# NOAA-GFDL/GFDL_atmos_cubed_sphere

Hardware: AMD Instinct MI355X
Metric: c_sw+d_sw cell-updates/s (higher is better)
Workload: dtype f64; 1 GPU; doubly periodic 384x384x127 tile per GPU (C384L127-sized), nonhydrostatic, c_sw+d_sw pair, hord 10/10/10/10, nord=1, d4_bg=0.16; layout=1x1, halo=periodic copy, gridstruct=orthogonal + uniform (metric terms as scalars), build_id=3496e67435bd, launch=eager launches

## Files before the change

### gfdl_atmos_cubed_sphere_amd/csrc/csw_march.h

```cpp
#pragma once

#include "csw_kernel.h"
#include "tp2d_march.h"

namespace fv3 {

constexpr int kCswCols = 58;
constexpr int kCswLast = 60;

inline MarchDims make_csw_dims(const Grid &g, int tj) {
  MarchDims d;
  d.tj = tj;
  d.klist = nullptr;
  d.nk = 0;
  d.k_fast = 0;
  d.nstrips = (g.nx + 4 + kCswCols - 1) / kCswCols;
  d.nsegs = (g.ny + 4 + tj - 1) / tj;
  d.alt_nk = d.alt_ng = d.alt_tj = 0;
  d.set_box(0, d.nstrips, 0, d.nsegs);
  return d;
}

struct CswMetrics {
  vd cs, rs, cosau, rsinu, dy, sg3, sg1, dx, sg4, sg2, dxc, dyc, rac, fc;
  vd ra, sinau, rdxc, cosav, sinav, rdyc;
};
struct CswFields {
  vd u, v, dp, pt, w;
};

struct CswLevel {
  vd u0, u1, u2, u3;
  vd v0, v1, v2, v3;
// ... 12 lines not shown
  }
};

template <int KPW, int GM = 0, bool CS = false>
struct CswMarch {
#ifdef FV3_CSW_TWO_WAVES
  static constexpr int kTwoWavesPerSimd = 1;
#endif
  Grid g;
  CswArgs a;
  MarchDims md;
  int nkg;

  FV3_D void operator()(int gid) const {
    constexpr double a1 = 0.5625, a2 = -0.0625;
    int strip, seg, kg, tjw;
    md.decode_tj(gid, strip, seg, kg, tjw);
    const int is = g.is, ie = g.ie, js = g.js, je = g.je;
    const int ilo = is - 1 + strip * kCswCols - 3;
    auto cl = [](int v, int lo, int hi) { return v < lo ? lo : (v > hi ? hi : v); };
    const vl cA = make_lanes(cl(g.isd - ilo, 0, kW - 1), cl(g.ied - ilo, 0, kW - 1));
    const vl cV = make_lanes(cl(g.isd - ilo, 0, kW - 1), cl(g.ied + 1 - ilo, 0, kW - 1));
    int l2 = cl(ie + 2 - ilo, 0, kCswLast), l1 = cl(ie + 1 - ilo, 0, kCswLast);
    const int mw = CS ? a.mask_w : 0;
    const int l0 = mw ? (3 > mw + 1 - ilo ? 3 : mw + 1 - ilo) : 3;
    if (mw) {
      const int lm = g.npx - mw - 1 - ilo;
      l2 = l2 < lm ? l2 : lm;
      l1 = l1 < lm ? l1 : lm;
    }
    const int oJ0 = mw ? mw + 1 : g.jsd - 1, oJ1 = mw ? g.npy - mw - 1 : g.jed + 2;
    const int jA = js - 1 + seg * tjw;
    const int jB = (jA + tjw - 1 < je + 2) ? jA + tjw - 1 : je + 2;
    const bool nh = !a.hydrostatic;
    const double dt2 = a.dt2, dt4 = 0.5 * dt2;
    const long nAp = (long)g.nA();
    auto LA = [&](const double *p, int j, long shift = 0) { return vload(p, (long)g.iA(ilo, cl(j, g.jsd, g.jed)) + shift, cA); };
    auto LU = [&](const double *p, int j) { return vload(p, (long)g.iU(ilo, cl(j, g.jsd, g.jed + 1)), cA); };
    auto LV = [&](const double *p, int j) { return vload(p, (long)g.iV(ilo, cl(j, g.jsd, g.jed)), cV); };
    auto LB = [&](const double *p, int j) { return vload(p, (long)g.iB(ilo, cl(j, g.jsd, g.jed + 1)), cV); };
    const vb m_uc = lane_mask(is - ilo, ie + 1 - ilo);
    const vb m_vc = lane_mask(is - ilo, ie - ilo);
    const vm s1 = make_mask(l0, l1), s2 = make_mask(l0, l2);

    int kl[KPW];
    bool live[KPW];
    for (int m = 0; m < KPW; m++) {
      const int k = kg * KPW + m;
// ... 174 lines not shown
```

### gfdl_atmos_cubed_sphere_amd/csrc/dsw_fused.h

```cpp
#pragma once

#include "dsw_march.h"

#ifndef FV3_BF
#define FV3_BF 1
#endif
#ifndef FV3_MOM_3W
#define FV3_MOM_3W 1
#endif

namespace fv3 {

struct Tp2dShared {
  vd cx, xf, ar, rax;
  vd cy, yf;
  vd arj, cxj, ray;
  vd rrax, rray;
};

template <int HORD>
struct Tp2dField {
  static constexpr int ORD_IN = (HORD == 10) ? 8 : HORD;
  static constexpr int ORD_OU = HORD;
  PpmY<ORD_IN> ya;
// ... 43 lines not shown
    vd cy, yf;
    vd xfj, ra;
    vd ucj;
    vd rdxa, dyr, sg3, sg1;
    vd rdya0, rdya1, dxr, sg4, sg2;
  };

  FV3_D void operator()(int gid) const {
    if constexpr (FLUXES || !FV3_BF)
      run_general(gid);
    else
      run_bf(gid);
  }

  FV3_D void run_bf(int gid) const {
    int strip, seg, kk, tjw;
    md.decode_tj(gid, strip, seg, kk, tjw);
    const int k = md.klist ? md.klist[kk] : kk;
    const StripGeom s = make_strip(g, strip);
    const int ilo = s.ilo;
    const int jA = g.js + seg * tjw;
    const int jB = (jA + tjw - 1 < g.je) ? jA + tjw - 1 : g.je;
    const int rlast = jB + 3;
    const int lFx1 = (ilo + s.lC1 == g.ie) ? s.lC1 + 1 : s.lC1;
    const size_t oA = (size_t)k * g.nA(), oCX = (size_t)k * g.nCX(), oCY = (size_t)k * g.nCY();
    const size_t oFX = (size_t)k * g.nFX(), oFY = (size_t)k * g.nFY(), oCC = (size_t)k * g.nCC();
    const double *delp = a.delp + oA, *pt = a.pt + oA, *w = NH ? a.w + oA : nullptr;
    double *crx = a.crx + oCX, *xfx = a.xfx + oCX, *cry = a.cry + oCY, *yfx = a.yfx + oCY;
    double *mfx = a.mfx + oFX, *mfy = a.mfy + oFY;
    const int seg_last = (jB == g.je);
    const int rowA = (seg == 0) ? g.jsd : jA, rowB = seg_last ? g.jed : jB;
    const int lY0 = (strip == 0) ? s.lA0 : s.lC0, lY1 = (ilo + s.lC1 == g.ie) ? s.lA1 : s.lC1;
    const double dt = a.dt;
    const int mw = a.mask_w;
    const int oC0 = mw ? (s.lC0 > mw + 1 - ilo ? s.lC0 : mw + 1 - ilo) : s.lC0;
    const int oC1 = mw ? (s.lC1 < g.npx - mw - 1 - ilo ? s.lC1 : g.npx - mw - 1 - ilo) : s.lC1;
    const int oF1 = mw ? (lFx1 < g.npx - mw - 1 - ilo ? lFx1 : g.npx - mw - 1 - ilo) : lFx1;
    const int oJ0 = mw ? mw + 1 : g.jsd, oJ1 = mw ? g.npy - mw - 1 : g.jed + 1;
    const vm mCX = make_mask(s.lC0, lFx1), mCY = make_mask(lY0, lY1), mO = make_mask(oC0, oC1), mOF = make_mask(oC0, oF1),
             mC = make_mask(s.lC0, s.lC1);
    const bool wdamp = UNI && NH && a.lv.damp_w[k] > 1.E-5;
    const double damp4 = wdamp ? a.lv.damp_w[k] * g.da_min_c : 0., dd8 = a.kgb * fabs(a.dt);

    auto load_in = [&](int r) {
      In in;
      const long iA = (long)g.iA(ilo, r), iCX = (long)g.iCX(ilo, r);
// ... 359 lines not shown

  struct In {
    vd u1, v0, v1, dx1, dy0, dy1, ra, f0;
    vd ar, cx, xf, cy, yf;
    vd vc, uc, ukc, rdy, rdx, dv, dgu, dgv, rac;
  };

  FV3_D void operator()(int gid) const {
    if constexpr (FV3_BF)
      run_bf(gid);
    else
      run_general(gid);
  }

  FV3_D void run_bf(int gid) const {
    int strip, seg, kk, tjw;
    md.decode_tj(gid, strip, seg, kk, tjw);
    const int k = md.klist ? md.klist[kk] : kk;
    const StripGeom s = make_strip(g, strip);
    const int ilo = s.ilo;
    const int jA = g.js + seg * tjw;
    const int jB = (jA + tjw - 1 < g.je) ? jA + tjw - 1 : g.je;
    const int rlast = jB + 3;
    const int lFx1 = (ilo + s.lC1 == g.ie) ? s.lC1 + 1 : s.lC1;
    const double *u = a.u + (size_t)k * g.nU(), *v = a.v + (size_t)k * g.nV();
    const double *uc = a.uc + (size_t)k * g.nV(), *vc = a.vc + (size_t)k * g.nU();
    const double *dv = a.divg_d + (size_t)k * g.nB();
    const double *crx = a.crx + (size_t)k * g.nCX(), *xfx = a.xfx + (size_t)k * g.nCX();
    const double *cry = a.cry + (size_t)k * g.nCY(), *yfx = a.yfx + (size_t)k * g.nCY();
    double *uo = a.u_out + (size_t)k * g.nU(), *vo = a.v_out + (size_t)k * g.nV();
    double *dpc = a.delpc ? a.delpc + (size_t)k * g.nA() : nullptr;
    const double dt5 = 0.5 * a.dt, dt = a.dt;
    const int mw = CS ? a.mask_w : 0;
    const int oC0 = (CS && mw) ? (s.lC0 > mw + 1 - ilo ? s.lC0 : mw + 1 - ilo) : s.lC0;
    const int oC1 = (CS && mw) ? (s.lC1 < g.npx - mw - 1 - ilo ? s.lC1 : g.npx - mw - 1 - ilo) : s.lC1;
    const int oF1 = (CS && mw) ? (lFx1 < g.npx - mw - 1 - ilo ? lFx1 : g.npx - mw - 1 - ilo) : lFx1;
    const int oJ0 = (CS && mw) ? mw + 1 : g.jsd, oJ1 = (CS && mw) ? g.npy - mw - 1 : g.jed + 1;
// ... 431 lines not shown
```

### gfdl_atmos_cubed_sphere_amd/csrc/fv3_api.hip

```cpp
#include "../../include/fv3_mi355x.h"

#include <algorithm>
#include <cstdarg>
#include <deque>
#include <unordered_map>
#include <new>
#include <type_traits>

#include "csw_kernel.h"
#include "csw_march.h"
#include "cubed_csw.h"
#include "cubed_tp.h"
#include "cubed_tpf.h"
#include "cube_topo.h"
#include "cubed_dsw.h"
#include "cubed_damp.h"
#include "cubed_a2b.h"
#include "dsw_kernels.h"
#include "dsw_march.h"
#include "dsw_fused.h"
#include "fv3_common.h"
#include "fv3_launch.h"
#include "nh_kernels.h"
#include "nh_fast.h"
#include "nh_alt.h"
#include "neg_adj.h"
#include "subgrid_z.h"
#include "phys_update.h"
#include "held_suarez.h"
#include "reed_phys.h"
#include "kessler_phys.h"
#include "diag_kernels.h"
#include "remap_kernels.h"
#include "remap_fast.h"
#include "tracer_kernels.h"
// ... 13 lines not shown
struct CubePlanDev;
constexpr int kMarchTj = 48;
struct fv3_ctx {
  fv3_domain dom = {};
  Grid g = {};
  stream_t stream = {};
  stream_t stream2 = {};
  void *ev_fork = nullptr, *ev_join = nullptr;
  int lane = 0;
  void *ev_mid = nullptr;
  bool side_ok = false;
  struct LevSel { int *klist, *klist_m; int n_plain, n_damp, n_plain_m, n_rest_m; bool side_ok; } lev_sel[2] = {};
  int use_side = 1;
  int sponge_march = 1;
  int round_simds = 0;
  double *dev_metrics = nullptr;
  bool grid_ready = false;
  int *lev_i = nullptr;
  double *lev_d = nullptr;
  bool lev_ready = false;
  double *dp0 = nullptr;
  double *edge_dev = nullptr;
  EdgeCoef ec = {};
  bool dp0_ready = false;
  double *scratch[8] = {};
  double *ray_d = nullptr;
  struct RegEntry { const void *host; void *dev; size_t bytes; bool dev_current, host_current; };
  std::vector<RegEntry> *reg = nullptr;
  int reg_lazy = 0;
  long long reg_stat[4] = {};
// ... 498 lines not shown
  g.is = dom->is; g.ie = dom->ie; g.js = dom->js; g.je = dom->je;
  g.isd = dom->is - NG; g.ied = dom->ie + NG; g.jsd = dom->js - NG; g.jed = dom->je + NG;
  g.npx = dom->npx; g.npy = dom->npy; g.npz = dom->npz;
  g.nid = g.ied - g.isd + 1; g.njd = g.jed - g.jsd + 1; g.nx = g.ie - g.is + 1; g.ny = g.je - g.js + 1;
  g.grid_type = dom->grid_type;
  g.do_diss_est = dom->do_diss_est; g.prevent_diss_cooling = dom->prevent_diss_cooling;
  g.stretched_grid = dom->stretched_grid;
  g.lim_fac = dom->lim_fac;
  ctx_switches(c);
  *out = c;
  return 0;
}

extern "C" int fv3_comm_destroy(fv3_ctx *c);
static void cube_plans_free(fv3_ctx *c);
extern "C" int fv3_destroy(fv3_ctx *c) {
  if (!c) return 0;
  if (c->grp) {
    fv3_group *g = c->grp;
    (void)grp_pump(g, true);
    for (int m = 0; m < g->n; m++)
      if (g->m[m] == c) g->m[m] = nullptr;
    for (int m = 0; m < g->n; m++)
      if (g->m[m]) g->m[m]->grp = nullptr;
    g->n = 0;
    c->grp = nullptr;
  }
  const int guards = c->poison ? work_check_guards(c, "fv3_destroy") : 0;
  cube_plans_free(c);
  fv3_comm_destroy(c);
  if (c->dev_metrics) rt_free(c->dev_metrics);
  if (c->lev_i) rt_free(c->lev_i);
  if (c->lev_d) rt_free(c->lev_d);
  if (c->dp0) rt_free(c->dp0);
  if (c->akbk) rt_free(c->akbk);
  work_free(c, &c->remap_scr);
  if (c->ray_d) rt_free(c->ray_d);
  if (c->rff_d) rt_free(c->rff_d);
  delete c->reg;
  work_free(c, &c->trc_d);
  if (c->trc_i) rt_free(c->trc_i);
  if (c->ones_i) rt_free(c->ones_i);
  if (c->kord_tr_dev) rt_free(c->kord_tr_dev);
  if (c->edge_dev) rt_free(c->edge_dev);
  if (c->lev_ext_d) rt_free(c->lev_ext_d);
// ... 178 lines not shown
  RT(grp_stream_op(c, 2, dst, src, bytes, 0));
  return 0;
}
extern "C" int fv3_memset(fv3_ctx *c, void *dst, int value, size_t bytes) {
  RT(grp_stream_op(c, 1, dst, nullptr, bytes, value));
  return 0;
}
extern "C" int fv3_sync(fv3_ctx *c) {
  RT(rtf_sync(c ? c->stream : nullptr));
  if (c && c->poison) return work_check_guards(c, "fv3_sync");
  return 0;
}

extern "C" int fv3_grid_upload(fv3_ctx *c, const fv3_grid_host *h) {
  if (!c || !h) return fail("fv3_grid_upload: null argument");
  c->host_area.clear();
  c->global_area = 0.;
  Grid &g = c->g;
  const size_t nA = g.nA(), nU = g.nU(), nV = g.nV(), nB = g.nB();
  struct Item { const double *src; const double **dst; size_t n; };
  Item items[] = {
      {h->area, &g.area, nA}, {h->rarea, &g.rarea, nA}, {h->dxa, &g.dxa, nA}, {h->dya, &g.dya, nA},
      {h->rdxa, &g.rdxa, nA}, {h->rdya, &g.rdya, nA}, {h->cosa_s, &g.cosa_s, nA}, {h->rsin2, &g.rsin2, nA},
      {h->f0, &g.f0, nA},
      {h->dx, &g.dx, nU}, {h->rdx, &g.rdx, nU}, {h->dyc, &g.dyc, nU}, {h->rdyc, &g.rdyc, nU},
      {h->cosa_v, &g.cosa_v, nU}, {h->sina_v, &g.sina_v, nU}, {h->rsin_v, &g.rsin_v, nU},
      {h->divg_u, &g.divg_u, nU}, {h->del6_u, &g.del6_u, nU},
      {h->dy, &g.dy, nV}, {h->rdy, &g.rdy, nV}, {h->dxc, &g.dxc, nV}, {h->rdxc, &g.rdxc, nV},
      {h->cosa_u, &g.cosa_u, nV}, {h->sina_u, &g.sina_u, nV}, {h->rsin_u, &g.rsin_u, nV},
      {h->divg_v, &g.divg_v, nV}, {h->del6_v, &g.del6_v, nV},
// ... 44 lines not shown
  return 0;
}

extern "C" int fv3_grid_geom(const fv3_ctx *c) { return (c && c->grid_ready) ? c->g.geom : -1; }

static void lev_activate(fv3_ctx *c, int x) {
  const fv3_ctx::LevSel &ls = c->lev_sel[x];
  c->klist = ls.klist; c->n_plain = ls.n_plain; c->n_damp = ls.n_damp;
  c->klist_m = ls.klist_m; c->n_plain_m = ls.n_plain_m; c->n_rest_m = ls.n_rest_m;
  c->side_ok = ls.side_ok;
}

extern "C" int fv3_dsw_levels_upload(fv3_ctx *c, const fv3_dsw_levels *lv) {
  if (!c || !lv) return fail("fv3_dsw_levels_upload: null argument");
  const int npz = c->g.npz;
  if (!c->lev_i) RT(rt_malloc((void **)&c->lev_i, sizeof(int) * 4 * npz));
  if (!c->lev_d) RT(rt_malloc((void **)&c->lev_d, sizeof(double) * 5 * npz));
  const int *iv[4] = {lv->nord_k, lv->nord_v, lv->nord_w, lv->nord_t};
  const double *dv[5] = {lv->d2_divg, lv->damp_vt, lv->damp_w, lv->damp_t, lv->d_con_k};
  for (int n = 0; n < 4; n++) {
    for (int k = 0; k < npz; k++) {
      if (iv[n][k] < 0 || iv[n][k] > (n == 0 ? 3 : 2)) return fail("fv3_dsw_levels_upload: nord out of range at k=%d", k);
    }
    RT(rtf_h2d(c->lev_i + n * npz, iv[n], sizeof(int) * npz, c->stream));
  }
  for (int n = 0; n < 5; n++) RT(rtf_h2d(c->lev_d + n * npz, dv[n], sizeof(double) * npz, c->stream));
  {
    std::vector<int> ni(npz + 1);
    std::vector<double> nd(npz + 1);
    for (int k = 0; k < npz; k++) { ni[k] = lv->nord_v[k]; nd[k] = lv->damp_vt[k]; }
// ... 451 lines not shown
    case 11: RT(launch_w(c, "ppm_line", 1, PpmLineMarch<11>{h, cr, flux, n, which - 1})); break;
    case 12: RT(launch_w(c, "ppm_line", 1, PpmLineMarch<12>{h, cr, flux, n, which - 1})); break;
    case 1: RT(launch_w(c, "ppm_line", 1, PpmLineMarchLin<1>{h, cr, flux, n, which - 1, c->g.lim_fac})); break;
    case -1: RT(launch_w(c, "ppm_line", 1, PpmLineMarchLin<-1>{h, cr, flux, n, which - 1, c->g.lim_fac})); break;
    case 2: RT(launch_w(c, "ppm_line", 1, PpmLineMarchLin<2>{h, cr, flux, n, which - 1, c->g.lim_fac})); break;
    case -2: RT(launch_w(c, "ppm_line", 1, PpmLineMarchLin<-2>{h, cr, flux, n, which - 1, c->g.lim_fac})); break;
    case 3: RT(launch_w(c, "ppm_line", 1, PpmLineMarchLin<3>{h, cr, flux, n, which - 1, c->g.lim_fac})); break;
    case -3: RT(launch_w(c, "ppm_line", 1, PpmLineMarchLin<-3>{h, cr, flux, n, which - 1, c->g.lim_fac})); break;
    case 4: RT(launch_w(c, "ppm_line", 1, PpmLineMarchLin<4>{h, cr, flux, n, which - 1, c->g.lim_fac})); break;
    case -4: RT(launch_w(c, "ppm_line", 1, PpmLineMarchLin<-4>{h, cr, flux, n, which - 1, c->g.lim_fac})); break;
    default: return fail("fv3_ppm_line: hord=%d not supported -- " FV3_HORD_TABLE, iord);
  }
  return 0;
}

static void seg_report(const char *who, const MarchDims &d, int nlev) {
  static const int on = env_int("FV3_MI355X_DEBUG_SEGMENTS", 0);
  if (on)
    std::fprintf(stderr, "[fv3 segments] %s: %d level slots x %d strips x %d segments of %d rows; %d of the slots (spread evenly): %d segments of %d rows\n", who, nlev,
                 d.nstrips, d.nsegs, d.tj, d.alt_nk, d.alt_ng, d.alt_tj);
}
static int seg_rows(const fv3_ctx *c, int tj_conf, int nlev_slots) {
  const Grid &g = c->g;
  if (c->tj_fixed) return tj_conf;
  const int nstrips = num_strips(g);
  const long have = (long)nstrips * (nlev_slots > 0 ? nlev_slots : 1);
  const int want_segs = (int)((2048 + have - 1) / have);
  int tj = (g.ny + want_segs - 1) / want_segs;
  if (tj < 8) tj = 8;
  return tj < tj_conf ? tj : tj_conf;
}

template <class F>
static int dispatch_geom(int geom, F &&f) {
  switch (geom) {
    case 2: return f(std::integral_constant<int, 2>{});
    case 1: return f(std::integral_constant<int, 1>{});
    default: return f(std::integral_constant<int, 0>{});
  }
}

extern "C" int fv3_c_sw(fv3_ctx *c, double *delpc, const double *delp, double *ptc, const double *pt,
                        const double *u, const double *v, const double *w, double *uc, double *vc, double *ua,
                        double *va, double *wc, double *ut, double *vt, double *divg_d, int nord, double dt2,
                        int hydrostatic, int dord4) {
// ... 11 lines not shown
  kf.g = c->g;
  kf.a = CswArgs{delpc, ptc, wc, uc, vc, ua, va, ut, vt, divg_d, delp, pt, u, v, w, nord, hydrostatic, dt2};
  Dim3 grid;
  CswTile<TI, TJ>::grid_dims(c->g, grid.x, grid.y);
  grid.z = (unsigned)c->g.npz;
  RT(launch_p(c, "c_sw", grid, CswTile<TI, TJ>::lds_doubles, kf));
  return 0;
}

static int csw_march(fv3_ctx *c, const CswArgs &ca) {
  {
    const bool uni = c->g.geom == 2;
    MarchDims md = make_csw_dims(c->g, seg_rows(c, uni ? 24 : 64, c->g.npz));
    const int kpw = uni ? 1 : 2;
    const int nkg = (c->g.npz + kpw - 1) / kpw;
    if (uni && ca.mask_w == 0)
      balance_segments(md, nkg, c->g.ny + 4, 4 * c->round_simds, md.tj);
    const int nw = md.nwaves(nkg);
    seg_report("c_sw", md, nkg);
    if (ca.mask_w > 0) {
      if (kpw == 1) return launch_w(c, "c_sw", nw, CswMarch<1, 0, true>{c->g, ca, md, nkg});
      return launch_w(c, "c_sw", nw, CswMarch<2, 0, true>{c->g, ca, md, nkg});
    }
    auto go = [&](auto GMc) -> int {
      constexpr int GM = decltype(GMc)::value;
      return launch_w(c, "c_sw", nw, CswMarch<(GM == 2 ? 1 : 2), GM>{c->g, ca, md, nkg});
    };
    return dispatch_geom(c->g.geom, go);
  }
}

template <class Fn>
static int dispatch_hord(int hord, Fn &&fn) {
  switch (hord) {
// ... 66 lines not shown
    const int NS = mf.nstrips, NG = mf.nsegs;
    auto fused_launch = [&](int nwf) -> int {
      return dispatch_hord(a.hord_dp, [&](auto H) {
        constexpr int HORD = decltype(H)::value;
        if (g.geom == 2) {
          if (a.hydrostatic) return launch_w(c, "d_sw_fused", nwf, DswTransportFused<HORD, false, true, 2>{g, a, mf});
          return launch_w(c, "d_sw_fused", nwf, DswTransportFused<HORD, true, true, 2>{g, a, mf});
        }
        if (a.hydrostatic) return launch_w(c, "d_sw_fused", nwf, DswTransportFused<HORD, false, true>{g, a, mf});
        return launch_w(c, "d_sw_fused", nwf, DswTransportFused<HORD, true, true>{g, a, mf});
      });
    };
    auto box = [&](int s0, int ns, int g0, int ng) -> int {
      if (ns <= 0 || ng <= 0) return 0;
      mf.set_box(s0, ns, g0, ng);
      if (FV3_BF && s0 == 0 && ns == NS && g0 == 0 && ng == NG && a.mask_w == 0)
        balance_segments(mf, c->n_plain, g.ny, 2 * c->round_simds, mf.tj);
      seg_report("d_sw_fused", mf, c->n_plain);
      return fused_launch(mf.nwaves(c->n_plain));
    };
    if (region == 0 || !dsw_has_interior(c)) return region == 1 ? 0 : box(0, NS, 0, NG);
    if (region == 1) return box(1, NS - 2, 1, NG - 2);
    mf.set_frame();
    return fused_launch(mf.nwaves(c->n_plain));
  }
  if (region == 1) return 0;
  double *fxs = c->mflux[0], *fys = c->mflux[1];
  int rc = dispatch_hord_all(a.hord_dp, [&](auto H) {
    DswDelpMarch<decltype(H)::value> kf{g, a, md, fxs, fys, 1};
    return launch_w(c, "d_sw_delp", nw, kf);
  });
  if (rc) return rc;
  auto scalar = [&](const char *label, int hord, const double *q, double *q_out) {
    return dispatch_hord_all(hord, [&](auto H) {
// ... 1 lines not shown
      return launch_w(c, label, nw, kf);
    });
  };
  if (!a.hydrostatic && (rc = scalar("d_sw_w", a.hord_vt, a.w, a.w_out))) return rc;
  if (a.use_cond && (rc = scalar("d_sw_qcon", a.hord_dp, a.q_con, a.q_con_out))) return rc;
  return scalar("d_sw_pt", a.hord_tm, a.pt, a.pt_out);
}

static int dsw_momentum_march(fv3_ctx *c, const DswArgs &a, int part = 0) {
  const Grid &g = c->g;
  const bool fused_m = dsw_momentum_fused(c, a);
  if (!fused_m && !c->ke_scr) RT(work_alloc(c, "ke_scr", 0, &c->ke_scr, g.nB() * g.npz));
  if (fused_m) {
    MarchDims mf = make_march_dims(g, seg_rows(c, (a.mask_w && !c->tj_env_fused) ? 55 : c->march_tj_fused, g.npz));
    mf.klist = c->klist_m;
    if (FV3_BF && a.mask_w == 0)
      balance_segments(mf, c->n_plain_m, g.ny, ((g.geom == 2 && FV3_MOM_3W) ? 3 : 2) * c->round_simds, mf.tj);
    const int nwf = mf.nwaves(c->n_plain_m);
    seg_report("d_sw_mom_fused", mf, c->n_plain_m);
    return dispatch_hord(a.hord_vt, [&](auto H) {
      constexpr int HORD = decltype(H)::value;
      if (g.geom == 2) {
        switch (sw_class(a.hord_mt)) {
          case 5: return launch_w(c, "d_sw_mom_fused", nwf, DswMomentumFused<5, HORD, 2>{g, a, mf});
          case 6: return launch_w(c, "d_sw_mom_fused", nwf, DswMomentumFused<6, HORD, 2>{g, a, mf});
          default: return launch_w(c, "d_sw_mom_fused", nwf, DswMomentumFused<8, HORD, 2>{g, a, mf});
        }
      }
      if (a.rsina) {
        switch (sw_class_cubed(a.hord_mt)) {
          case 5: return launch_w(c, "d_sw_mom_fused", nwf, DswMomentumFused<5, HORD, 0, true>{g, a, mf});
          case 6: return launch_w(c, "d_sw_mom_fused", nwf, DswMomentumFused<6, HORD, 0, true>{g, a, mf});
          case 108: return launch_w(c, "d_sw_mom_fused", nwf, DswMomentumFused<108, HORD, 0, true>{g, a, mf});
          case 110: return launch_w(c, "d_sw_mom_fused", nwf, DswMomentumFused<110, HORD, 0, true>{g, a, mf});
// ... 3196 lines not shown
```

### gfdl_atmos_cubed_sphere_amd/csrc/tp2d_march.h

```cpp
#pragma once

#include <type_traits>

#include <cstdlib>

#include "ppm_march.h"

namespace fv3 {

constexpr int kStripCells = kW - 6;

struct StripGeom {
  int ilo;
  int lA0, lA1;
  int lF0, lF1;
  int lC0, lC1;
  vl A, F, C;
};

FV3_D StripGeom make_strip(const Grid &g, int strip) {
  StripGeom s;
  const int ic0 = g.is + strip * kStripCells;
  s.ilo = ic0 - 3;
  auto clampi = [](int v, int lo, int hi) { return v < lo ? lo : (v > hi ? hi : v); };
  s.lA0 = clampi(g.isd - s.ilo, 0, kW - 1);
  s.lA1 = clampi(g.ied - s.ilo, 0, kW - 1);
  s.lF0 = clampi(g.is - s.ilo, 0, kW - 1);
  s.lF1 = clampi(g.ie + 1 - s.ilo, 0, kW - 1);
  s.lC0 = 3;
  s.lC1 = clampi(g.ie - s.ilo, 0, kW - 4);
  s.A = make_lanes(s.lA0, s.lA1);
  s.F = make_lanes(s.lF0, s.lF1);
  s.C = make_lanes(s.lC0, s.lC1);
  return s;
}
inline int num_strips(const Grid &g) { return (g.nx + kStripCells - 1) / kStripCells; }

struct MarchDims {
  int nstrips, nsegs, tj;
  const int *klist;
  int nk;
  int k_fast;
  int s0, ns, g0, ng;
  int frame;
  int alt_nk, alt_ng, alt_tj;
  FV3_HD void set_box(int s0_, int ns_, int g0_, int ng_) { s0 = s0_; ns = ns_; g0 = g0_; ng = ng_; frame = 0; }
  FV3_HD void set_frame() { s0 = 0; ns = nstrips; g0 = 0; ng = nsegs; frame = 1; }
  FV3_HD int ncells() const { return frame ? nstrips * nsegs - (nstrips - 2) * (nsegs - 2) : ns * ng; }
  FV3_HD int alt_before(int kk) const { return (int)(((long)kk * alt_nk) / nk); }
  FV3_HD int waves_before(int kk) const { return nstrips * (kk * nsegs - alt_before(kk) * (nsegs - alt_ng)); }
  FV3_HD int nwaves(int npz) {
    nk = npz;
    if (alt_nk > npz) alt_nk = npz;
    if (frame || ns != nstrips || ng != nsegs || k_fast) alt_nk = 0;
    if (alt_nk > 0) return waves_before(npz);
    return ncells() * npz;
  }
  FV3_HD void decode_tj(int gid, int &strip, int &seg, int &kk, int &tjw) const {
    tjw = tj;
    if (alt_nk > 0) {
      int lo = 0, hi = nk;
      while (hi - lo > 1) {
        const int mid = (lo + hi) >> 1;
        if (waves_before(mid) <= gid) lo = mid; else hi = mid;
      }
      kk = lo;
      const int r = gid - waves_before(kk);
      const bool alt = alt_before(kk + 1) > alt_before(kk);
      if (alt) tjw = alt_tj;
      strip = r % nstrips;
      seg = r / nstrips;
      return;
    }
    decode(gid, strip, seg, kk);
  }
  FV3_HD void frame_cell(int t, int &strip, int &seg) const {
    if (t < nstrips) { strip = t; seg = 0; return; }
    t -= nstrips;
    if (t < nstrips) { strip = t; seg = nsegs - 1; return; }
    t -= nstrips;
    if (t < nsegs - 2) { strip = 0; seg = 1 + t; return; }
    t -= nsegs - 2;
    strip = nstrips - 1;
    seg = 1 + t;
  }
  FV3_HD void decode(int gid, int &strip, int &seg, int &kk) const {
    if (frame) {
      const int nc = ncells();
      kk = gid / nc;
// ... 6 lines not shown
    } else {
      strip = s0 + gid % ns;
      seg = g0 + (gid / ns) % ng;
      kk = gid / (ns * ng);
    }
  }
};
inline MarchDims make_march_dims(const Grid &g, int tj) {
  MarchDims d;
  d.tj = tj;
  d.klist = nullptr;
  d.nk = 0;
  d.k_fast = 0;
  d.nstrips = num_strips(g);
  d.nsegs = (g.ny + tj - 1) / tj;
  d.alt_nk = d.alt_ng = d.alt_tj = 0;
  d.set_box(0, d.nstrips, 0, d.nsegs);
  return d;
}

inline void balance_segments(MarchDims &d, int nlev, int rows, int round_waves, int tj_conf) {
  d.alt_nk = 0;
  const int S = (rows + tj_conf - 1) / tj_conf;
  d.tj = (rows + S - 1) / S;
  d.nsegs = (rows + d.tj - 1) / d.tj;
  d.set_box(0, d.nstrips, 0, d.nsegs);
  if (nlev <= 0 || round_waves <= 0 || d.nsegs < 2) return;
  const long total = (long)nlev * d.nstrips * d.nsegs;
  const long whole = total / round_waves, excess = total - whole * round_waves;
  if (whole < 1 || excess == 0 || excess * 4 > round_waves) return;
  const int tjA = (rows + d.nsegs - 2) / (d.nsegs - 1);
  if ((rows + tjA - 1) / tjA != d.nsegs - 1) return;
  const long margin = round_waves / 64;
  const int L = (int)((excess + margin + d.nstrips - 1) / d.nstrips);
  if (2 * L > nlev) return;
  d.alt_nk = L;
  d.alt_ng = d.nsegs - 1;
  d.alt_tj = tjA;
}

struct MarchIn {
  vd qn, ar, cx, xf;
  vd cy, yf;
};

template <int HORD, bool UNI_AREA = false>
struct Tp2dState {
  static constexpr int ORD_IN = (HORD == 10) ? 8 : HORD;
  static constexpr int ORD_OU = HORD;
  PpmY<ORD_IN> ya;
  PpmY<ORD_OU> yb;
  vd fx2_0, fx2_1, fx2_2, fx2_3;
  vd fy2y_prev, yf_prev, fyv_prev;
// ... 130 lines not shown
```

### include/fv3_mi355x.h

```cpp
#ifndef FV3_MI355X_H
#define FV3_MI355X_H

#include <stddef.h>

#ifdef __cplusplus
extern "C" {
#endif

typedef struct fv3_ctx fv3_ctx;

typedef struct fv3_domain {
  int is, ie, js, je;
  int ng;
  int npx, npy, npz;
  int grid_type;
  int do_diss_est, prevent_diss_cooling, stretched_grid;
  double lim_fac;
} fv3_domain;

typedef struct fv3_grid_host {
  double da_min, da_min_c;
  const double *area, *rarea, *dxa, *dya, *rdxa, *rdya, *cosa_s, *rsin2, *f0;
  const double *dx, *rdx, *dyc, *rdyc, *cosa_v, *sina_v, *rsin_v, *divg_u, *del6_u;
  const double *dy, *rdy, *dxc, *rdxc, *cosa_u, *sina_u, *rsin_u, *divg_v, *del6_v;
// ... 9 lines not shown
  const double *ec1, *ec2, *en1, *en2;
} fv3_grid_cubed;

const char *fv3_last_error(void);
int fv3_create(const fv3_domain *dom, fv3_ctx **out);
int fv3_destroy(fv3_ctx *ctx);
int fv3_set_stream(fv3_ctx *ctx, void *stream);
int fv3_grid_upload(fv3_ctx *ctx, const fv3_grid_host *g);
typedef struct fv3_group fv3_group;
int fv3_group_create(fv3_ctx *const *members, int n, fv3_group **out);
int fv3_group_flush(fv3_group *grp);
int fv3_group_stats(fv3_group *grp, long *merged, long *single);
int fv3_group_destroy(fv3_group *grp);
int fv3_grid_upload_cubed(fv3_ctx *ctx, const fv3_grid_cubed *g);
int fv3_grid_geom(const fv3_ctx *ctx);

int fv3_malloc(void **dptr, size_t bytes);
int fv3_free(void *dptr);
int fv3_memcpy_h2d(fv3_ctx *ctx, void *dst, const void *src, size_t bytes);
int fv3_memcpy_d2h(fv3_ctx *ctx, void *dst, const void *src, size_t bytes);
int fv3_memset(fv3_ctx *ctx, void *dst, int value, size_t bytes);
int fv3_memcpy_d2d(fv3_ctx *ctx, void *dst, const void *src, size_t bytes);
int fv3_sync(fv3_ctx *ctx);

int fv3_registry_mode(fv3_ctx *ctx, int lazy);
int fv3_registry_put(fv3_ctx *ctx, void *dev, const void *host, size_t bytes);
int fv3_registry_get(fv3_ctx *ctx, void *host, const void *dev, size_t bytes);
int fv3_registry_host_touched(fv3_ctx *ctx, const void *host);
int fv3_registry_fetch(fv3_ctx *ctx, void *host);
int fv3_registry_forget(fv3_ctx *ctx, void *host, int discard);
// ... 324 lines not shown
```

Measured before the change: 10.76 billion cell-updates/s.

## Replace segment balancing with host-planned per-wave piece tables for march kernels

```diff
diff --git a/gfdl_atmos_cubed_sphere_amd/csrc/csw_march.h b/gfdl_atmos_cubed_sphere_amd/csrc/csw_march.h
--- a/gfdl_atmos_cubed_sphere_amd/csrc/csw_march.h
+++ b/gfdl_atmos_cubed_sphere_amd/csrc/csw_march.h
@@ -16,7 +16,7 @@
   d.k_fast = 0;
   d.nstrips = (g.nx + 4 + kCswCols - 1) / kCswCols;
   d.nsegs = (g.ny + 4 + tj - 1) / tj;
-  d.alt_nk = d.alt_ng = d.alt_tj = 0;
+  d.pieces = nullptr;
   d.set_box(0, d.nstrips, 0, d.nsegs);
   return d;
 }
@@ -59,8 +59,8 @@
 
   FV3_D void operator()(int gid) const {
     constexpr double a1 = 0.5625, a2 = -0.0625;
-    int strip, seg, kg, tjw;
-    md.decode_tj(gid, strip, seg, kg, tjw);
+    int strip, kg, jA, jB;
+    if constexpr (CS) md.rows_of(gid, g.js - 1, g.je + 2, strip, kg, jA, jB); else md.rows_planned(gid, g.js - 1, strip, kg, jA, jB);
     const int is = g.is, ie = g.ie, js = g.js, je = g.je;
     const int ilo = is - 1 + strip * kCswCols - 3;
     auto cl = [](int v, int lo, int hi) { return v < lo ? lo : (v > hi ? hi : v); };
@@ -75,8 +75,6 @@
       l1 = l1 < lm ? l1 : lm;
     }
     const int oJ0 = mw ? mw + 1 : g.jsd - 1, oJ1 = mw ? g.npy - mw - 1 : g.jed + 2;
-    const int jA = js - 1 + seg * tjw;
-    const int jB = (jA + tjw - 1 < je + 2) ? jA + tjw - 1 : je + 2;
     const bool nh = !a.hydrostatic;
     const double dt2 = a.dt2, dt4 = 0.5 * dt2;
     const long nAp = (long)g.nA();
diff --git a/gfdl_atmos_cubed_sphere_amd/csrc/dsw_fused.h b/gfdl_atmos_cubed_sphere_amd/csrc/dsw_fused.h
--- a/gfdl_atmos_cubed_sphere_amd/csrc/dsw_fused.h
+++ b/gfdl_atmos_cubed_sphere_amd/csrc/dsw_fused.h
@@ -81,13 +81,11 @@
   }
 
   FV3_D void run_bf(int gid) const {
-    int strip, seg, kk, tjw;
-    md.decode_tj(gid, strip, seg, kk, tjw);
+    int strip, kk, jA, jB;
+    md.rows_of(gid, g.js, g.je, strip, kk, jA, jB);
     const int k = md.klist ? md.klist[kk] : kk;
     const StripGeom s = make_strip(g, strip);
     const int ilo = s.ilo;
-    const int jA = g.js + seg * tjw;
-    const int jB = (jA + tjw - 1 < g.je) ? jA + tjw - 1 : g.je;
     const int rlast = jB + 3;
     const int lFx1 = (ilo + s.lC1 == g.ie) ? s.lC1 + 1 : s.lC1;
     const size_t oA = (size_t)k * g.nA(), oCX = (size_t)k * g.nCX(), oCY = (size_t)k * g.nCY();
@@ -96,7 +94,7 @@
     double *crx = a.crx + oCX, *xfx = a.xfx + oCX, *cry = a.cry + oCY, *yfx = a.yfx + oCY;
     double *mfx = a.mfx + oFX, *mfy = a.mfy + oFY;
     const int seg_last = (jB == g.je);
-    const int rowA = (seg == 0) ? g.jsd : jA, rowB = seg_last ? g.jed : jB;
+    const int rowA = (jA == g.js) ? g.jsd : jA, rowB = seg_last ? g.jed : jB;
     const int lY0 = (strip == 0) ? s.lA0 : s.lC0, lY1 = (ilo + s.lC1 == g.ie) ? s.lA1 : s.lC1;
     const double dt = a.dt;
     const int mw = a.mask_w;
@@ -486,13 +484,11 @@
   }
 
   FV3_D void run_bf(int gid) const {
-    int strip, seg, kk, tjw;
-    md.decode_tj(gid, strip, seg, kk, tjw);
+    int strip, kk, jA, jB;
+    if constexpr (CS) md.rows_of(gid, g.js, g.je, strip, kk, jA, jB); else md.rows_planned(gid, g.js, strip, kk, jA, jB);
     const int k = md.klist ? md.klist[kk] : kk;
     const StripGeom s = make_strip(g, strip);
     const int ilo = s.ilo;
-    const int jA = g.js + seg * tjw;
-    const int jB = (jA + tjw - 1 < g.je) ? jA + tjw - 1 : g.je;
     const int rlast = jB + 3;
     const int lFx1 = (ilo + s.lC1 == g.ie) ? s.lC1 + 1 : s.lC1;
     const double *u = a.u + (size_t)k * g.nU(), *v = a.v + (size_t)k * g.nV();
diff --git a/gfdl_atmos_cubed_sphere_amd/csrc/fv3_api.hip b/gfdl_atmos_cubed_sphere_amd/csrc/fv3_api.hip
--- a/gfdl_atmos_cubed_sphere_amd/csrc/fv3_api.hip
+++ b/gfdl_atmos_cubed_sphere_amd/csrc/fv3_api.hip
@@ -19,6 +19,7 @@
 #include "dsw_kernels.h"
 #include "dsw_march.h"
 #include "dsw_fused.h"
+#include "march_plan.h"
 #include "fv3_common.h"
 #include "fv3_launch.h"
 #include "nh_kernels.h"
@@ -62,6 +63,8 @@
   int use_side = 1;
   int sponge_march = 1;
   int round_simds = 0;
+  struct MarchTable { int key[6]; MarchPiece *dev; int n, makespan; std::string lengths; };
+  std::vector<MarchTable> march_tables;
   double *dev_metrics = nullptr;
   bool grid_ready = false;
   int *lev_i = nullptr;
@@ -590,6 +593,13 @@
 
 extern "C" int fv3_comm_destroy(fv3_ctx *c);
 static void cube_plans_free(fv3_ctx *c);
+static void march_tables_drop(fv3_ctx *c) {
+  if (c->march_tables.empty()) return;
+  (void)grp_flush_all();
+  (void)rt_sync(c->stream);
+  for (auto &t : c->march_tables) rt_free(t.dev);
+  c->march_tables.clear();
+}
 extern "C" int fv3_destroy(fv3_ctx *c) {
   if (!c) return 0;
   if (c->grp) {
@@ -605,6 +615,7 @@
   const int guards = c->poison ? work_check_guards(c, "fv3_destroy") : 0;
   cube_plans_free(c);
   fv3_comm_destroy(c);
+  for (auto &t : c->march_tables) rt_free(t.dev);
   if (c->dev_metrics) rt_free(c->dev_metrics);
   if (c->lev_i) rt_free(c->lev_i);
   if (c->lev_d) rt_free(c->lev_d);
@@ -813,6 +824,7 @@
 
 extern "C" int fv3_grid_upload(fv3_ctx *c, const fv3_grid_host *h) {
   if (!c || !h) return fail("fv3_grid_upload: null argument");
+  march_tables_drop(c);
   c->host_area.clear();
   c->global_area = 0.;
   Grid &g = c->g;
@@ -887,6 +899,7 @@
 extern "C" int fv3_dsw_levels_upload(fv3_ctx *c, const fv3_dsw_levels *lv) {
   if (!c || !lv) return fail("fv3_dsw_levels_upload: null argument");
   const int npz = c->g.npz;
+  march_tables_drop(c);
   if (!c->lev_i) RT(rt_malloc((void **)&c->lev_i, sizeof(int) * 4 * npz));
   if (!c->lev_d) RT(rt_malloc((void **)&c->lev_d, sizeof(double) * 5 * npz));
   const int *iv[4] = {lv->nord_k, lv->nord_v, lv->nord_w, lv->nord_t};
@@ -1368,21 +1381,78 @@
   return 0;
 }
 
-static void seg_report(const char *who, const MarchDims &d, int nlev) {
+static const fv3_ctx::MarchTable *march_table(fv3_ctx *c, int kernel, const MarchPlanSpec &sp) {
+  const int key[6] = {kernel, sp.rows, sp.nstrips, sp.nlev, sp.slots > 0 ? sp.slots : 0, sp.tj};
+  for (const auto &t : c->march_tables)
+    if (std::equal(key, key + 6, t.key)) return &t;
+  const MarchPlan plan = march_plan(sp);
+  if (plan.pieces.empty()) { fail("march_table: a launch of %d strips x %d level slots x %d rows has no plan", sp.nstrips, sp.nlev, sp.rows); return nullptr; }
+  fv3_ctx::MarchTable t;
+  std::copy(key, key + 6, t.key);
+  t.n = (int)plan.pieces.size();
+  t.makespan = plan.makespan;
+  t.lengths = march_plan_lengths(plan.pieces);
+  t.dev = nullptr;
+  const size_t bytes = sizeof(MarchPiece) * plan.pieces.size();
+  if (rt_malloc((void **)&t.dev, bytes) || rtf_h2d(t.dev, plan.pieces.data(), bytes, c->stream) || rtf_sync(c->stream)) {
+    if (t.dev) rt_free(t.dev);
+    fail("march_table: the table of %d pieces could not be uploaded", t.n);
+    return nullptr;
+  }
+  c->march_tables.push_back(t);
+  return &c->march_tables.back();
+}
+constexpr bool kPlanKernel[3] = {false, false, true};
+static int plan_slots(const fv3_ctx *c, int kernel, int waves_per_simd) {
+  return (c->tj_fixed || !kPlanKernel[kernel]) ? 0 : waves_per_simd * c->round_simds;
+}
+
+static void seg_report(const char *who, const MarchDims &d, int nlev, const fv3_ctx::MarchTable *t = nullptr) {
   static const int on = env_int("FV3_MI355X_DEBUG_SEGMENTS", 0);
-  if (on)
-    std::fprintf(stderr, "[fv3 segments] %s: %d level slots x %d strips x %d segments of %d rows; %d of the slots (spread evenly): %d segments of %d rows\n", who, nlev,
-                 d.nstrips, d.nsegs, d.tj, d.alt_nk, d.alt_ng, d.alt_tj);
-}
-static int seg_rows(const fv3_ctx *c, int tj_conf, int nlev_slots) {
-  const Grid &g = c->g;
-  if (c->tj_fixed) return tj_conf;
-  const int nstrips = num_strips(g);
+  if (!on) return;
+  if (t)
+    std::fprintf(stderr, "[fv3 segments] %s: %d level slots x %d strips, %s for %d resident wavefronts: %d pieces (%s), modelled makespan %d steps\n", who,
+                 nlev, d.nstrips, t->key[4] > 0 ? "planned" : "equal segments", t->key[4], t->n, t->lengths.c_str(), t->makespan);
+  else
+    std::fprintf(stderr, "[fv3 segments] %s: %d level slots x %d strips x %d segments of %d rows\n", who, nlev, d.nstrips, d.nsegs, d.tj);
+}
+static int seg_rows_of(int nx, int ny, int tj_conf, int nlev_slots) {
+  const int nstrips = (nx + kStripCells - 1) / kStripCells;
   const long have = (long)nstrips * (nlev_slots > 0 ? nlev_slots : 1);
   const int want_segs = (int)((2048 + have - 1) / have);
-  int tj = (g.ny + want_segs - 1) / want_segs;
+  int tj = (ny + want_segs - 1) / want_segs;
   if (tj < 8) tj = 8;
   return tj < tj_conf ? tj : tj_conf;
+}
+static int seg_rows(const fv3_ctx *c, int tj_conf, int nlev_slots) {
+  if (c->tj_fixed) return tj_conf;
+  return seg_rows_of(c->g.nx, c->g.ny, tj_conf, nlev_slots);
+}
+
+static int equal_rows(int rows, int tj_conf) {
+  const int S = (rows + tj_conf - 1) / tj_conf;
+  return (rows + S - 1) / S;
+}
+
+extern "C" int fv3_march_plan(int kernel, int nx, int ny, int level_slots, int resident, int cap, int *pieces, int *count, int *makespan) {
+  if (kernel < 0 || kernel > 2 || nx < 1 || ny < 1 || level_slots < 1 || !pieces || !count || !makespan) return fail("fv3_march_plan: bad argument");
+  MarchPlanSpec sp;
+  sp.nstrips = kernel == 0 ? (nx + 4 + kCswCols - 1) / kCswCols : (nx + kStripCells - 1) / kStripCells;
+  sp.nlev = level_slots;
+  sp.rows = kernel == 0 ? ny + 4 : ny;
+  sp.warm = kernel == 0 ? 6 : 7;
+  sp.slots = resident;
+  sp.tj = equal_rows(sp.rows, seg_rows_of(nx, ny, kernel == 0 ? 24 : kMarchTj, level_slots));
+  const MarchPlan plan = march_plan(sp);
+  if (plan.pieces.empty()) return fail("fv3_march_plan: no plan for this shape");
+  *count = (int)plan.pieces.size();
+  *makespan = plan.makespan;
+  if (*count > cap) return fail("fv3_march_plan: %d pieces, room for %d", *count, cap);
+  for (size_t n = 0; n < plan.pieces.size(); n++) {
+    const MarchPiece &q = plan.pieces[n];
+    pieces[4 * n] = q.strip; pieces[4 * n + 1] = q.slot; pieces[4 * n + 2] = q.ja; pieces[4 * n + 3] = q.jb;
+  }
+  return 0;
 }
 
 template <class F>
@@ -1424,10 +1494,16 @@
     MarchDims md = make_csw_dims(c->g, seg_rows(c, uni ? 24 : 64, c->g.npz));
     const int kpw = uni ? 1 : 2;
     const int nkg = (c->g.npz + kpw - 1) / kpw;
-    if (uni && ca.mask_w == 0)
-      balance_segments(md, nkg, c->g.ny + 4, 4 * c->round_simds, md.tj);
-    const int nw = md.nwaves(nkg);
-    seg_report("c_sw", md, nkg);
+    int nw = md.nwaves(nkg);
+    const fv3_ctx::MarchTable *tab = nullptr;
+    if (ca.mask_w == 0) {
+      const int rows = c->g.ny + 4;
+      tab = march_table(c, 0, MarchPlanSpec{md.nstrips, nkg, rows, 6, uni ? plan_slots(c, 0, 4) : 0, uni ? equal_rows(rows, md.tj) : md.tj});
+      if (!tab) return 1;
+      md.pieces = tab->dev;
+      nw = tab->n;
+    }
+    seg_report("c_sw", md, nkg, tab);
     if (ca.mask_w > 0) {
       if (kpw == 1) return launch_w(c, "c_sw", nw, CswMarch<1, 0, true>{c->g, ca, md, nkg});
       return launch_w(c, "c_sw", nw, CswMarch<2, 0, true>{c->g, ca, md, nkg});
@@ -1524,10 +1600,16 @@
     auto box = [&](int s0, int ns, int g0, int ng) -> int {
       if (ns <= 0 || ng <= 0) return 0;
       mf.set_box(s0, ns, g0, ng);
-      if (FV3_BF && s0 == 0 && ns == NS && g0 == 0 && ng == NG && a.mask_w == 0)
-        balance_segments(mf, c->n_plain, g.ny, 2 * c->round_simds, mf.tj);
-      seg_report("d_sw_fused", mf, c->n_plain);
-      return fused_launch(mf.nwaves(c->n_plain));
+      int nwf = mf.nwaves(c->n_plain);
+      const fv3_ctx::MarchTable *tab = nullptr;
+      if (FV3_BF && s0 == 0 && ns == NS && g0 == 0 && ng == NG && a.mask_w == 0) {
+        tab = march_table(c, 1, MarchPlanSpec{NS, c->n_plain, g.ny, 7, plan_slots(c, 1, 2), equal_rows(g.ny, mf.tj)});
+        if (!tab) return 1;
+        mf.pieces = tab->dev;
+        nwf = tab->n;
+      }
+      seg_report("d_sw_fused", mf, c->n_plain, tab);
+      return fused_launch(nwf);
     };
     if (region == 0 || !dsw_has_interior(c)) return region == 1 ? 0 : box(0, NS, 0, NG);
     if (region == 1) return box(1, NS - 2, 1, NG - 2);
@@ -1559,10 +1641,16 @@
   if (fused_m) {
     MarchDims mf = make_march_dims(g, seg_rows(c, (a.mask_w && !c->tj_env_fused) ? 55 : c->march_tj_fused, g.npz));
     mf.klist = c->klist_m;
-    if (FV3_BF && a.mask_w == 0)
-      balance_segments(mf, c->n_plain_m, g.ny, ((g.geom == 2 && FV3_MOM_3W) ? 3 : 2) * c->round_simds, mf.tj);
-    const int nwf = mf.nwaves(c->n_plain_m);
-    seg_report("d_sw_mom_fused", mf, c->n_plain_m);
+    int nwf = mf.nwaves(c->n_plain_m);
+    const fv3_ctx::MarchTable *tab = nullptr;
+    if (FV3_BF && (a.mask_w == 0 || g.geom == 2 || !a.rsina)) {
+      tab = march_table(c, 2, MarchPlanSpec{mf.nstrips, c->n_plain_m, g.ny, 7, plan_slots(c, 2, (g.geom == 2 && FV3_MOM_3W) ? 3 : 2),
+                                            equal_rows(g.ny, mf.tj)});
+      if (!tab) return 1;
+      mf.pieces = tab->dev;
+      nwf = tab->n;
+    }
+    seg_report("d_sw_mom_fused", mf, c->n_plain_m, tab);
     return dispatch_hord(a.hord_vt, [&](auto H) {
       constexpr int HORD = decltype(H)::value;
       if (g.geom == 2) {
diff --git a/gfdl_atmos_cubed_sphere_amd/csrc/march_plan.h b/gfdl_atmos_cubed_sphere_amd/csrc/march_plan.h
--- /dev/null
+++ b/gfdl_atmos_cubed_sphere_amd/csrc/march_plan.h
@@ -0,0 +1,159 @@
+#pragma once
+
+#include <algorithm>
+#include <cstdio>
+#include <functional>
+#include <string>
+#include <vector>
+
+#include "tp2d_march.h"
+
+namespace fv3 {
+
+#ifndef FV3_HOST_EMU
+static_assert(kNT == 256, "march_plan.h counts four wavefronts per workgroup, as launch_waves does");
+#endif
+constexpr int kPlanMinRows = 8;
+constexpr int kPlanXcds = 8;
+
+struct MarchPlanSpec {
+  int nstrips, nlev, rows;
+  int warm;
+  int slots;
+  int tj;
+};
+struct MarchPlan {
+  std::vector<MarchPiece> pieces;
+  int makespan = 0;
+};
+
+inline int march_range_waves(int n) {
+  const int nblocks = (n + 3) / 4;
+  if (nblocks < 4 * kPlanXcds) return 0;
+  return 4 * ((nblocks + kPlanXcds - 1) / kPlanXcds);
+}
+
+inline int march_makespan(const MarchPiece *p, int n, int slots, int warm) {
+  const int rw = march_range_waves(n);
+  const int nranges = rw ? kPlanXcds : 1, machines = std::max(1, slots / nranges);
+  int worst = 0;
+  std::vector<int> heap;
+  for (int x = 0; x < nranges; x++) {
+    const int b = rw ? std::min(n, x * rw) : 0, e = rw ? std::min(n, (x + 1) * rw) : n;
+    heap.assign((size_t)std::min(machines, e - b), 0);
+    for (int i = b; i < e; i++) {
+      std::pop_heap(heap.begin(), heap.end(), std::greater<int>());
+      const int t = heap.back() + (int)p[i].jb - (int)p[i].ja + 1 + warm;
+      heap.back() = t;
+      std::push_heap(heap.begin(), heap.end(), std::greater<int>());
+      worst = std::max(worst, t);
+    }
+  }
+  return worst;
+}
+
+inline void march_plan_equal(const MarchPlanSpec &s, std::vector<MarchPiece> &out) {
+  const int tj = std::max(1, s.tj), nsegs = (s.rows + tj - 1) / tj;
+  out.clear();
+  out.reserve((size_t)s.nlev * nsegs * s.nstrips);
+  for (int k = 0; k < s.nlev; k++)
+    for (int g = 0; g < nsegs; g++)
+      for (int i = 0; i < s.nstrips; i++)
+        out.push_back(MarchPiece{(unsigned short)i, (unsigned short)k, (unsigned short)(g * tj),
+                                 (unsigned short)std::min(g * tj + tj - 1, s.rows - 1)});
+}
+
+inline bool march_plan_build(const MarchPlanSpec &s, int nl, int sh, std::vector<MarchPiece> &out) {
+  const int R = s.rows, ncol = s.nstrips * s.nlev;
+  if (nl < 1 || sh < 0) return false;
+  if ((nl > 1 || sh > 0) && (R - sh) / nl < kPlanMinRows) return false;
+  if (sh > 0 && (sh < kPlanMinRows || sh > (R - sh) / nl)) return false;
+  const int extra = sh > 0 ? (4 - (int)(((long)ncol * nl) % 4)) % 4 : 0;
+  if (extra > 0 && (extra > ncol || R / (nl + 1) < kPlanMinRows)) return false;
+  auto is_extra = [&](int col) { return col >= ncol - extra; };
+  std::vector<MarchPiece> lg, st;
+  lg.reserve((size_t)ncol * nl + extra);
+  st.reserve(sh > 0 ? (size_t)ncol : 0);
+  for (int k = 0; k < s.nlev; k++) {
+    for (int p = 0; p <= nl; p++)
+      for (int i = 0; i < s.nstrips; i++) {
+        const int col = k * s.nstrips + i;
+        const int np = is_extra(col) ? nl + 1 : nl, span = is_extra(col) ? R : R - sh;
+        if (p >= np) continue;
+        const int a = (int)((long)span * p / np), b = (int)((long)span * (p + 1) / np) - 1;
+        lg.push_back(MarchPiece{(unsigned short)i, (unsigned short)k, (unsigned short)a, (unsigned short)b});
+      }
+    if (sh > 0)
+      for (int i = 0; i < s.nstrips; i++)
+        if (!is_extra(k * s.nstrips + i))
+          st.push_back(MarchPiece{(unsigned short)i, (unsigned short)k, (unsigned short)(R - sh), (unsigned short)(R - 1)});
+  }
+  const long NL = (long)lg.size(), NS = (long)st.size(), n = NL + NS;
+  out.clear();
+  out.reserve((size_t)n);
+  const int rw = march_range_waves((int)n);
+  const int nranges = rw ? kPlanXcds : 1;
+  long doneL = 0, doneS = 0;
+  for (int x = 0; x < nranges; x++) {
+    const long e = (x == nranges - 1) ? n : std::min(n, (long)(x + 1) * rw);
+    long cumL = NL;
+    if (e < n) {
+      cumL = (NL * e / n) & ~3L;
+      const long lo = std::max(doneL, (std::max(0L, e - NS) + 3) & ~3L), hi = std::min(NL & ~3L, e - doneS);
+      cumL = std::max(lo, std::min(hi, cumL));
+    }
+    for (; doneL < cumL; doneL++) out.push_back(lg[(size_t)doneL]);
+    for (; doneL + doneS < e; doneS++) out.push_back(st[(size_t)doneS]);
+  }
+  return (long)out.size() == n;
+}
+
+inline MarchPlan march_plan(const MarchPlanSpec &s) {
+  MarchPlan best;
+  if (s.nstrips < 1 || s.nlev < 1 || s.rows < 1 || s.nstrips > 65535 || s.nlev > 65535 || s.rows > 65535) return best;
+  march_plan_equal(s, best.pieces);
+  best.makespan = march_makespan(best.pieces.data(), (int)best.pieces.size(), std::max(1, s.slots), s.warm);
+  if (s.slots <= 0) return best;
+  const int ncol = s.nstrips * s.nlev, m = s.slots / ncol;
+  const int nsegs = (s.rows + std::max(1, s.tj) - 1) / std::max(1, s.tj);
+  const int nlmax = std::max(1, s.rows / kPlanMinRows);
+  int nls[5] = {m - 1, m, m + 1, m + 2, nsegs};
+  for (int &nl : nls) nl = std::max(1, std::min(nlmax, nl));
+  std::vector<MarchPiece> cand;
+  bool first = true;
+  for (int c = 0; c < 5; c++) {
+    const int nl = nls[c];
+    bool seen = false;
+    for (int d = 0; d < c; d++) seen = seen || nls[d] == nl;
+    if (seen) continue;
+    for (int sh = 0; sh <= s.rows / (nl + 1); sh = sh ? sh + 1 : kPlanMinRows) {
+      if (!march_plan_build(s, nl, sh, cand)) continue;
+      const int ms = march_makespan(cand.data(), (int)cand.size(), s.slots, s.warm);
+      const bool better = first ? ms <= best.makespan : (ms < best.makespan || (ms == best.makespan && cand.size() < best.pieces.size()));
+      if (better) {
+        best.pieces.swap(cand);
+        best.makespan = ms;
+        first = false;
+      }
+    }
+  }
+  return best;
+}
+
+inline std::string march_plan_lengths(const std::vector<MarchPiece> &p) {
+  std::vector<int> len;
+  for (const MarchPiece &q : p) len.push_back((int)q.jb - (int)q.ja + 1);
+  std::sort(len.begin(), len.end(), std::greater<int>());
+  std::string out;
+  for (size_t i = 0; i < len.size();) {
+    size_t j = i;
+    while (j < len.size() && len[j] == len[i]) j++;
+    char buf[64];
+    std::snprintf(buf, sizeof buf, "%s%zu x %d rows", out.empty() ? "" : ", ", j - i, len[i]);
+    out += buf;
+    i = j;
+  }
+  return out;
+}
+
+}
diff --git a/gfdl_atmos_cubed_sphere_amd/csrc/tp2d_march.h b/gfdl_atmos_cubed_sphere_amd/csrc/tp2d_march.h
--- a/gfdl_atmos_cubed_sphere_amd/csrc/tp2d_march.h
+++ b/gfdl_atmos_cubed_sphere_amd/csrc/tp2d_march.h
@@ -36,6 +36,10 @@
 }
 inline int num_strips(const Grid &g) { return (g.nx + kStripCells - 1) / kStripCells; }
 
+struct alignas(8) MarchPiece {
+  unsigned short strip, slot, ja, jb;
+};
+
 struct MarchDims {
   int nstrips, nsegs, tj;
   const int *klist;
@@ -43,36 +47,28 @@
   int k_fast;
   int s0, ns, g0, ng;
   int frame;
-  int alt_nk, alt_ng, alt_tj;
+  const MarchPiece *pieces;
   FV3_HD void set_box(int s0_, int ns_, int g0_, int ng_) { s0 = s0_; ns = ns_; g0 = g0_; ng = ng_; frame = 0; }
   FV3_HD void set_frame() { s0 = 0; ns = nstrips; g0 = 0; ng = nsegs; frame = 1; }
   FV3_HD int ncells() const { return frame ? nstrips * nsegs - (nstrips - 2) * (nsegs - 2) : ns * ng; }
-  FV3_HD int alt_before(int kk) const { return (int)(((long)kk * alt_nk) / nk); }
-  FV3_HD int waves_before(int kk) const { return nstrips * (kk * nsegs - alt_before(kk) * (nsegs - alt_ng)); }
   FV3_HD int nwaves(int npz) {
     nk = npz;
-    if (alt_nk > npz) alt_nk = npz;
-    if (frame || ns != nstrips || ng != nsegs || k_fast) alt_nk = 0;
-    if (alt_nk > 0) return waves_before(npz);
     return ncells() * npz;
   }
-  FV3_HD void decode_tj(int gid, int &strip, int &seg, int &kk, int &tjw) const {
-    tjw = tj;
-    if (alt_nk > 0) {
-      int lo = 0, hi = nk;
-      while (hi - lo > 1) {
-        const int mid = (lo + hi) >> 1;
-        if (waves_before(mid) <= gid) lo = mid; else hi = mid;
-      }
-      kk = lo;
-      const int r = gid - waves_before(kk);
-      const bool alt = alt_before(kk + 1) > alt_before(kk);
-      if (alt) tjw = alt_tj;
-      strip = r % nstrips;
-      seg = r / nstrips;
-      return;
-    }
+  FV3_HD void rows_planned(int gid, int j0, int &strip, int &kk, int &jA, int &jB) const {
+    unsigned long long p;
+    __builtin_memcpy(&p, pieces + gid, sizeof p);
+    strip = (int)(p & 0xffffu);
+    kk = (int)((p >> 16) & 0xffffu);
+    jA = j0 + (int)((p >> 32) & 0xffffu);
+    jB = j0 + (int)(p >> 48);
+  }
+  FV3_HD void rows_of(int gid, int j0, int j1, int &strip, int &kk, int &jA, int &jB) const {
+    if (pieces) { rows_planned(gid, j0, strip, kk, jA, jB); return; }
+    int seg;
     decode(gid, strip, seg, kk);
+    jA = j0 + seg * tj;
+    jB = (jA + tj - 1 < j1) ? jA + tj - 1 : j1;
   }
   FV3_HD void frame_cell(int t, int &strip, int &seg) const {
     if (t < nstrips) { strip = t; seg = 0; return; }
@@ -109,29 +105,9 @@
   d.k_fast = 0;
   d.nstrips = num_strips(g);
   d.nsegs = (g.ny + tj - 1) / tj;
-  d.alt_nk = d.alt_ng = d.alt_tj = 0;
+  d.pieces = nullptr;
   d.set_box(0, d.nstrips, 0, d.nsegs);
   return d;
-}
-
-inline void balance_segments(MarchDims &d, int nlev, int rows, int round_waves, int tj_conf) {
-  d.alt_nk = 0;
-  const int S = (rows + tj_conf - 1) / tj_conf;
-  d.tj = (rows + S - 1) / S;
-  d.nsegs = (rows + d.tj - 1) / d.tj;
-  d.set_box(0, d.nstrips, 0, d.nsegs);
-  if (nlev <= 0 || round_waves <= 0 || d.nsegs < 2) return;
-  const long total = (long)nlev * d.nstrips * d.nsegs;
-  const long whole = total / round_waves, excess = total - whole * round_waves;
-  if (whole < 1 || excess == 0 || excess * 4 > round_waves) return;
-  const int tjA = (rows + d.nsegs - 2) / (d.nsegs - 1);
-  if ((rows + tjA - 1) / tjA != d.nsegs - 1) return;
-  const long margin = round_waves / 64;
-  const int L = (int)((excess + margin + d.nstrips - 1) / d.nstrips);
-  if (2 * L > nlev) return;
-  d.alt_nk = L;
-  d.alt_ng = d.nsegs - 1;
-  d.alt_tj = tjA;
 }
 
 struct MarchIn {
diff --git a/include/fv3_mi355x.h b/include/fv3_mi355x.h
--- a/include/fv3_mi355x.h
+++ b/include/fv3_mi355x.h
@@ -47,6 +47,8 @@
 int fv3_group_destroy(fv3_group *grp);
 int fv3_grid_upload_cubed(fv3_ctx *ctx, const fv3_grid_cubed *g);
 int fv3_grid_geom(const fv3_ctx *ctx);
+
+int fv3_march_plan(int kernel, int nx, int ny, int level_slots, int resident, int cap, int *pieces, int *count, int *makespan);
 
 int fv3_malloc(void **dptr, size_t bytes);
 int fv3_free(void *dptr);
```

Measured after the change: 10.85 billion cell-updates/s, median of 6. About the same (+0.9%).
